# dcharatan/flowmap

Measured on NVIDIA B200. Metric: overfit iters/sec at 150x360x640 (149 frame pairs per iteration), higher is better.
Workload: dtype f32

## Files before the change

### flowmap_b200/csrc/fm_kernels.cu

```cuda
#include <cuda_runtime.h>
#include <stdio.h>
#include <string.h>
#include <stdlib.h>

#include "../../include/flowmap_b200.h"
#include "fm_host.h"
#include "fm_pixel.cuh"

namespace fm_host {
namespace {
thread_local char g_err[512] = "";
unsigned long long g_launches = 0;
}
int fail(const char* what, cudaError_t e) {
  snprintf(g_err, sizeof(g_err), "%s: %s", what, cudaGetErrorString(e));
  return 1;
}
int fail_msg(const char* what) {
  snprintf(g_err, sizeof(g_err), "%s", what);
  return 2;
}
void count_launch() { __atomic_add_fetch(&g_launches, 1, __ATOMIC_RELAXED); }
const char* last_error() { return g_err; }
unsigned long long launches() { return __atomic_load_n(&g_launches, __ATOMIC_RELAXED); }
// ... 1163 lines not shown
__device__ __forceinline__ Cam sm_cam(const float* rec) {
  Cam c;
  c.fx = rec1(rec, 15); c.fy = rec1(rec, 16); c.cx = rec1(rec, 17); c.cy = rec1(rec, 18);
  c.ifx = rec1(rec, 19); c.ify = rec1(rec, 20);
  return c;
}

template <int NT = kThreads>
__device__ __forceinline__ int block_compact(bool valid, int value, int* list, int* warp_base) {
  const int lane = threadIdx.x & 31, warp = threadIdx.x >> 5;
  const unsigned m = __ballot_sync(0xffffffffu, valid);
  if (lane == 0) warp_base[warp] = __popc(m);
  __syncthreads();
  int base = 0, total = 0;
#pragma unroll
  for (int w = 0; w < NT / 32; ++w) {
    const int c = warp_base[w];
    if (w < warp) base += c;
    total += c;
  }
  if (valid) list[base + __popc(m & ((1u << lane) - 1u))] = value;
  __syncthreads();
  return total;
}

struct TrackSlot { int slot; bool owner; };
template <int N, int OFF>
struct SlotWalk {
  __device__ __forceinline__ static void run(int lane, int& pos, bool& ok) {
    if (N == 1) {
      SlotWalk<1, OFF / 2>::run(lane, pos, ok);
      ok = ok && (lane & OFF) == 0;
    } else {
      constexpr int HALF = (N + 1) / 2;
      SlotWalk<HALF, OFF / 2>::run(lane, pos, ok);
      if (lane & OFF) pos += HALF;
      ok = ok && pos < N;
    }
  }
};
template <int N>
struct SlotWalk<N, 0> {
  __device__ __forceinline__ static void run(int, int& pos, bool& ok) { pos = 0; ok = true; }
};
template <int N>
__device__ __forceinline__ TrackSlot track_slot(int lane) {
  TrackSlot t;
  SlotWalk<N, 16>::run(lane, t.slot, t.owner);
  return t;
}
template <int N, int OFF>
__device__ __forceinline__ void halve_exchange(float* v, bool upper) {
  constexpr int HALF = (N + 1) / 2;
#pragma unroll
  for (int j = 0; j < HALF; ++j) {
    const float hi = (j + HALF < N) ? v[j + HALF] : 0.f;
    const float send = upper ? v[j] : hi;
    const float keep = upper ? hi : v[j];
    v[j] = keep + __shfl_xor_sync(0xffffffffu, send, OFF);
  }
}
template <int N, int OFF>
struct WarpSumN {
  __device__ __forceinline__ static void run(float* v, int lane) {
    if (N == 1) {
      v[0] += __shfl_xor_sync(0xffffffffu, v[0], OFF);
      WarpSumN<1, OFF / 2>::run(v, lane);
    } else {
      halve_exchange<N, OFF>(v, lane & OFF);
      WarpSumN<(N + 1) / 2, OFF / 2>::run(v, lane);
    }
  }
};
template <int N>
struct WarpSumN<N, 0> {
  __device__ __forceinline__ static void run(float*, int) {}
};
template <int N>
__device__ __forceinline__ float warp_sum_n(float* v, int lane) {
  WarpSumN<N, 16>::run(v, lane);
  return v[0];
}

constexpr int kTrackThreads = 128;
constexpr int kTrackPoints = 2 * kTrackThreads;

template <bool SHARED_K>
__global__ void __launch_bounds__(kTrackThreads, 5)
k_track_src(const float* __restrict__ depth, const float* __restrict__ k4, const float* __restrict__ ext,
            const int* __restrict__ seg, const float* __restrict__ txy,
            const unsigned char* __restrict__ tvis, int mapping, float delta, double* __restrict__ sums,
            unsigned char* __restrict__ flag, float* __restrict__ dq_out,
            double* __restrict__ trackacc, int H, int W, TrackShard sh) {
  extern __shared__ float sm[];
  constexpr int NW = kTrackThreads / 32;
  __shared__ double red[kTrackAcc * NW];
  const SegInfo si = load_seg(seg, blockIdx.z);
  const int row = blockIdx.y;
  if (row >= si.rows || !sh.owns(si.start_frame + row)) return;
  load_segment_frames(sm, ext, k4, si);
  float* s_tgt = sm + (size_t)gridDim.y * 2 * kTrackRec;
  __shared__ int s_list[kTrackPoints];
  __shared__ int s_wbase[NW];
  const GridDims grid = make_grid(H, W);
  const RobustCfg rc = make_robust(mapping, delta, H, W);
  const int frame = si.start_frame + row;
  const float* D = depth + (size_t)(frame - sh.depth_frame0) * H * W;
  const float* rsrec = sm + row * 2 * kTrackRec;
  float rs[12];
#pragma unroll
  for (int i = 0; i < 12; ++i) rs[i] = rec1(rsrec, i);
  const Cam ks = sm_cam(rsrec);
  const int lane = threadIdx.x & 31, warp = threadIdx.x >> 5;
  float acc[kTrackAcc], lc[2] = {0.f, 0.f};
#pragma unroll
  for (int i = 0; i < kTrackAcc; ++i) acc[i] = 0.f;
  int count = 0;
#pragma unroll
  for (int h = 0; h < 2; ++h) {
    const int p_own = blockIdx.x * kTrackPoints + h * kTrackThreads + (int)threadIdx.x;
    bool ok_own = false;
    if (p_own < si.n) {
      const size_t sidx = (size_t)si.sample_start + (size_t)row * si.n + p_own;
      const float2 sxy = __ldg(reinterpret_cast<const float2*>(txy) + sidx);
      ok_own = tvis[sidx] && in_unit_square(sxy.x, sxy.y);
      flag[sidx] = ok_own ? 1 : 0;
    }
    count += block_compact<kTrackThreads>(ok_own, p_own, s_list + count, s_wbase);
  }
  const int half = (count + 1) >> 1;
  const bool live_a = (int)threadIdx.x < half, live_b = (int)threadIdx.x + half < count;
  if (warp * 32 < half) {
    const int pa = live_a ? s_list[threadIdx.x] : 0, pb = live_b ? s_list[threadIdx.x + half] : 0;
    const size_t row0 = (size_t)si.sample_start + (size_t)row * si.n;
    float qa[3] = {0.f, 0.f, 0.f}, qb[3] = {0.f, 0.f, 0.f};
    F2 Xw[3] = {f2s(0.f), f2s(0.f), f2s(0.f)};
    auto lift = [&](int p, float* q, float* X) {
      const float2 sxy = __ldg(reinterpret_cast<const float2*>(txy) + row0 + p);
      const Taps t = bilinear_taps(sxy.x, sxy.y, grid);
      sample_surface(t, grid, ks, [D](int o) { return __ldg(D + o); }, q[0], q[1], q[2]);
#pragma unroll
      for (int i = 0; i < 3; ++i)
        X[i] = fm_fma(rs[i * 3 + 0], q[0], fm_fma(rs[i * 3 + 1], q[1], fm_fma(rs[i * 3 + 2], q[2], rs[9 + i])));
    };
    if (live_a) { float X[3]; lift(pa, qa, X); Xw[0].x = X[0]; Xw[1].x = X[1]; Xw[2].x = X[2]; }
    if (live_b) { float X[3]; lift(pb, qb, X); Xw[0].y = X[0]; Xw[1].y = X[1]; Xw[2].y = X[2]; }
    F2 G[3] = {f2s(0.f), f2s(0.f), f2s(0.f)}, lc2[2] = {f2s(0.f), f2s(0.f)};
    F2 kt[4] = {f2s(0.f), f2s(0.f), f2s(0.f), f2s(0.f)};
    constexpr int NRED = SHARED_K ? 6 : kTrackAcc;
    constexpr int SLOT0 = kTrackAcc - NRED;
    const TrackSlot slot = track_slot<NRED>(lane);
    float* tgt = s_tgt + (size_t)warp * si.rows * kTrackAcc;
    size_t ia = (size_t)si.sample_start + pa, ib = (size_t)si.sample_start + pb;
    unsigned char va_n = live_a ? tvis[ia] : 0, vb_n = live_b ? tvis[ib] : 0;
    float2 ga_n = live_a ? __ldg(reinterpret_cast<const float2*>(txy) + ia) : make_float2(0.f, 0.f);
    float2 gb_n = live_b ? __ldg(reinterpret_cast<const float2*>(txy) + ib) : make_float2(0.f, 0.f);
    for (int ft = 0; ft < si.rows; ++ft) {
      const unsigned char vis_a = va_n, vis_b = vb_n;
      const float2 ga = ga_n, gb = gb_n;
      if (ft + 1 < si.rows) {
        if (live_a) { ia += si.n; va_n = tvis[ia]; ga_n = __ldg(reinterpret_cast<const float2*>(txy) + ia); }
        if (live_b) { ib += si.n; vb_n = tvis[ib]; gb_n = __ldg(reinterpret_cast<const float2*>(txy) + ib); }
      }
      float c[NRED];
#pragma unroll
      for (int i = 0; i < NRED; ++i) c[i] = 0.f;
      bool ok = false;
      if (vis_a | vis_b) {
        const float* rec = sm + ft * 2 * kTrackRec;
        F2 R[9];
#pragma unroll
        for (int i = 0; i < 9; ++i) R[i] = rec2(rec, i);
        const F2 dir0 = f2_fma(R[0], Xw[0], f2_fma(R[3], Xw[1], f2_mul(R[6], Xw[2])));
        const F2 dir1 = f2_fma(R[1], Xw[0], f2_fma(R[4], Xw[1], f2_mul(R[7], Xw[2])));
        const F2 dir2 = f2_fma(R[2], Xw[0], f2_fma(R[5], Xw[1], f2_mul(R[8], Xw[2])));
        Cam2 kc;
        kc.fx = rec2(rec, 15); kc.fy = rec2(rec, 16); kc.cx = rec2(rec, 17); kc.cy = rec2(rec, 18);
        const LeanTerm2 lt = lean_term2(f2s(1.0f), dir0, dir1, dir2, rec2(rec, 12), rec2(rec, 13), rec2(rec, 14), kc,
                                        f2(ga.x, gb.x), f2(ga.y, gb.y), f2s(0.f), f2s(0.f), f2s(1.0f), rc);
        const bool oa = vis_a && in_unit_square(lt.uvx.x, lt.uvy.x);
        const bool ob = vis_b && in_unit_square(lt.uvx.y, lt.uvy.y);
        if (oa | ob) {
          ok = true;
          const F2 d0 = f2(oa ? lt.d0.x : 0.f, ob ? lt.d0.y : 0.f);
          const F2 d1 = f2(oa ? lt.d1.x : 0.f, ob ? lt.d1.y : 0.f);
          const F2 d2 = f2(oa ? lt.d2.x : 0.f, ob ? lt.d2.y : 0.f);
          lc2[0] = f2_add(lc2[0], f2(oa ? lt.loss.x : 0.f, ob ? lt.loss.y : 0.f));
          lc2[1] = f2_add(lc2[1], f2(oa ? 1.f : 0.f, ob ? 1.f : 0.f));
          const F2 g0 = f2_fma(R[0], d0, f2_fma(R[1], d1, f2_mul(R[2], d2)));
          const F2 g1 = f2_fma(R[3], d0, f2_fma(R[4], d1, f2_mul(R[5], d2)));
          const F2 g2 = f2_fma(R[6], d0, f2_fma(R[7], d1, f2_mul(R[8], d2)));
          G[0] = f2_add(G[0], g0); G[1] = f2_add(G[1], g1); G[2] = f2_add(G[2], g2);
          const F2 ex = f2_mul(d0, rec2(rec, 19)), ey = f2_mul(d1, rec2(rec, 20));
          if (SHARED_K) {
            kt[0] = f2_fma(ex, lt.P0, kt[0]); kt[1] = f2_fma(ey, lt.P1, kt[1]);
            kt[2] = f2_fma(ex, lt.P2, kt[2]); kt[3] = f2_fma(ey, lt.P2, kt[3]);
          } else {
            const F2 k0 = f2_mul(ex, lt.P0), k1 = f2_mul(ey, lt.P1), k2 = f2_mul(ex, lt.P2), k3 = f2_mul(ey, lt.P2);
            c[0] = k0.x + k0.y; c[1] = k1.x + k1.y; c[2] = k2.x + k2.y; c[3] = k3.x + k3.y;
          }
          const F2 e0 = f2_sub(Xw[0], rec2(rec, 9)), e1 = f2_sub(Xw[1], rec2(rec, 10)), e2 = f2_sub(Xw[2], rec2(rec, 11));
          const F2 t0 = f2_fma(e2, g1, f2_neg(f2_mul(e1, g2)));
          const F2 t1 = f2_fma(e0, g2, f2_neg(f2_mul(e2, g0)));
          const F2 t2 = f2_fma(e1, g0, f2_neg(f2_mul(e0, g1)));
          float* tw = c + (SHARED_K ? 0 : 4);
          tw[0] = t0.x + t0.y; tw[1] = t1.x + t1.y; tw[2] = t2.x + t2.y;
          tw[3] = -(g0.x + g0.y); tw[4] = -(g1.x + g1.y); tw[5] = -(g2.x + g2.y);
        }
      }
      float total = 0.f;
      if (__ballot_sync(0xffffffffu, ok)) total = warp_sum_n<NRED>(c, lane);
      if (slot.owner) tgt[ft * kTrackAcc + SLOT0 + slot.slot] = total;
    }
    lc[0] = lc2[0].x + lc2[0].y;
    lc[1] = lc2[1].x + lc2[1].y;
    auto finish = [&](int p, const float* q, float X0, float X1, float X2, float G0, float G1, float G2, float k0,
                      float k1, float k2, float k3) {
      const size_t sidx = row0 + p;
      const float dq0 = fm_fma(rs[0], G0, fm_fma(rs[3], G1, rs[6] * G2));
      const float dq1 = fm_fma(rs[1], G0, fm_fma(rs[4], G1, rs[7] * G2));
      const float dq2 = fm_fma(rs[2], G0, fm_fma(rs[5], G1, rs[8] * G2));
      dq_out[sidx * 3 + 0] = dq0; dq_out[sidx * 3 + 1] = dq1; dq_out[sidx * 3 + 2] = dq2;
      const float e0 = dq0 * ks.ifx, e1 = dq1 * ks.ify;
      acc[0] += k0 - e0 * q[0]; acc[1] += k1 - e1 * q[1]; acc[2] += k2 - e0 * q[2]; acc[3] += k3 - e1 * q[2];
      const float c0 = X0 - rs[9], c1 = X1 - rs[10], c2 = X2 - rs[11];
      acc[4] += c1 * G2 - c2 * G1;
      acc[5] += c2 * G0 - c0 * G2;
      acc[6] += c0 * G1 - c1 * G0;
      acc[7] += G0; acc[8] += G1; acc[9] += G2;
    };
    if (live_a) finish(pa, qa, Xw[0].x, Xw[1].x, Xw[2].x, G[0].x, G[1].x, G[2].x, kt[0].x, kt[1].x, kt[2].x, kt[3].x);
    if (live_b) finish(pb, qb, Xw[0].y, Xw[1].y, Xw[2].y, G[0].y, G[1].y, G[2].y, kt[0].y, kt[1].y, kt[2].y, kt[3].y);
  }
  block_accumulate<2, kTrackThreads>(lc, sums, red);
  block_accumulate<kTrackAcc, kTrackThreads>(acc, trackacc + (size_t)frame * kTrackAcc, red);
  const int live_warps = (half + 31) >> 5;
  for (int i = threadIdx.x; i < si.rows * kTrackAcc; i += kTrackThreads) {
    if (SHARED_K && i % kTrackAcc < 4) continue;
    double t = 0.0;
    for (int w = 0; w < live_warps; ++w) t += (double)s_tgt[(size_t)w * si.rows * kTrackAcc + i];
    if (t != 0.0) atomicAdd(trackacc + (size_t)si.start_frame * kTrackAcc + i, t);
  }
}

__device__ __forceinline__ double track_scale(const double* sums, float loss_weight, const float* go) {
  double cnt = sums[1];
  if (cnt == 0.0) cnt = 1.0;
  return (double)loss_weight * (go ? (double)*go : 1.0) / cnt;
}

__global__ void k_track_loss(const double* __restrict__ sums, float loss_weight, float* __restrict__ loss) {
  *loss = (float)(track_scale(sums, loss_weight, nullptr) * sums[0]);
}

__global__ void __launch_bounds__(kThreads)
k_track_apply(const float* __restrict__ k4, const int* __restrict__ seg, const float* __restrict__ txy,
              const unsigned char* __restrict__ flag, const float* __restrict__ dq,
              const double* __restrict__ sums, float loss_weight, const float* __restrict__ go,
              float* __restrict__ g_depth, int H, int W, TrackShard sh) {
  const SegInfo si = load_seg(seg, blockIdx.z);
  const int row = blockIdx.y;
  const int p = blockIdx.x * kThreads + threadIdx.x;
  if (row >= si.rows || p >= si.n || !sh.owns(si.start_frame + row)) return;
  const size_t sidx = (size_t)si.sample_start + (size_t)row * si.n + p;
  if (!flag[sidx]) return;
  const float scale = (float)track_scale(sums, loss_weight, go);
  const int frame = si.start_frame + row;
  const GridDims grid = make_grid(H, W);
  const Cam ks = make_cam(load_k4(k4, frame));
  const float2 sxy = __ldg(reinterpret_cast<const float2*>(txy) + sidx);
  const Taps t = bilinear_taps(sxy.x, sxy.y, grid);
  const float dq0 = scale * dq[sidx * 3 + 0], dq1 = scale * dq[sidx * 3 + 1], dq2 = scale * dq[sidx * 3 + 2];
  float rx0, ry0, rx1, ry1;
  tap_rays(t, grid, ks, rx0, ry0, rx1, ry1);
  float* gd = g_depth + (size_t)(frame - sh.depth_frame0) * H * W;
  red_add(gd + t.y0 * W + t.x0, t.w00 * (dq0 * rx0 + dq1 * ry0 + dq2));
  red_add(gd + t.y0 * W + t.x1, t.w01 * (dq0 * rx1 + dq1 * ry0 + dq2));
  red_add(gd + t.y1 * W + t.x0, t.w10 * (dq0 * rx0 + dq1 * ry1 + dq2));
  red_add(gd + t.y1 * W + t.x1, t.w11 * (dq0 * rx1 + dq1 * ry1 + dq2));
}

__global__ void k_track_finalize(const double* __restrict__ trackacc, const double* __restrict__ sums,
                                 float loss_weight, const float* __restrict__ go,
                                 const float* __restrict__ ext, float* __restrict__ g_ext,
                                 float* __restrict__ g_k4, int F) {
  const int f = blockIdx.x * blockDim.x + threadIdx.x;
  if (f >= F) return;
  const double sc = track_scale(sums, loss_weight, go);
  const double* a = trackacc + (size_t)f * kTrackAcc;
  for (int k = 0; k < 4; ++k) g_k4[(size_t)f * 4 + k] = (float)(sc * a[k]);
  const float* P = ext + (size_t)f * 16;
  const double w0 = 0.5 * sc * a[4], w1 = 0.5 * sc * a[5], w2 = 0.5 * sc * a[6];
  float* o = g_ext + (size_t)f * 16;
  for (int c = 0; c < 3; ++c) {
    const double r0 = P[0 * 4 + c], r1 = P[1 * 4 + c], r2 = P[2 * 4 + c];
    o[0 * 4 + c] = (float)(-w2 * r1 + w1 * r2);
    o[1 * 4 + c] = (float)(w2 * r0 - w0 * r2);
    o[2 * 4 + c] = (float)(-w1 * r0 + w0 * r1);
  }
  o[3] = (float)(sc * a[7]); o[7] = (float)(sc * a[8]); o[11] = (float)(sc * a[9]);
  o[12] = o[13] = o[14] = o[15] = 0.f;
}

constexpr int kSweepAcc = 80;

__global__ void k_sweep_base_k4(const float* __restrict__ cand_k4, float* __restrict__ base_k4, int B, int n) {
  const int t = blockIdx.x * blockDim.x + threadIdx.x;
  if (t >= B * 8) return;
  const int b = t >> 3, e = t & 7;
  base_k4[t] = cand_k4[(size_t)b * n * 8 + e];
}

__global__ void k_sweep_scale_solve(const double* __restrict__ base_moments, const float* __restrict__ depth,
                                    const float* __restrict__ cand_k4, float* __restrict__ rt,
                                    PairState* __restrict__ state, int B, int n, PairLayout lay, int H, int W) {
  const int item = blockIdx.x * blockDim.x + threadIdx.x;
  if (item >= B * n) return;
  const int b = item / n;
  const PairAddr pa = pair_addr(lay, item, H * W);
  const double z0 = (double)__ldg(depth + pa.depth_a + (size_t)H * W + (size_t)(H / 2) * W + W / 2);
  const double sx = (double)cand_k4[(size_t)b * n * 8 + 0] / (double)cand_k4[(size_t)item * 8 + 0];
  const double sy = (double)cand_k4[(size_t)b * n * 8 + 1] / (double)cand_k4[(size_t)item * 8 + 1];
  const double sc[3] = {sx, sy, 1.0};
  double m[kNumMoments];
  const double* bm = base_moments + (size_t)b * kNumMoments;
  m[0] = bm[0];
  for (int i = 0; i < 3; ++i) { m[1 + i] = bm[1 + i] * sc[i]; m[4 + i] = bm[4 + i] * sc[i]; }
  for (int a = 0; a < 3; ++a)
    for (int c = 0; c < 3; ++c) m[7 + a * 3 + c] = bm[7 + a * 3 + c] * sc[a] * sc[c];
  const double shift[3] = {0.0, 0.0, z0};
  PairState st;
  float out[12];
  procrustes_solve(m, shift, out, st);
  for (int k = 0; k < 12; ++k) rt[(size_t)item * 12 + k] = out[k];
  state[item] = st;
}

__global__ void k_sweep_aggregate(const PairAdjoint* __restrict__ adj, const float* __restrict__ cand_k4,
                                  PairAdjoint* __restrict__ out, int B, int n) {
  const int b = blockIdx.x, lane = threadIdx.x;
  double acc[16];
#pragma unroll
  for (int i = 0; i < 16; ++i) acc[i] = 0.0;
  for (int c = lane; c < n; c += 32) {
    const int item = b * n + c;
    const PairAdjoint a = adj[item];
    const double s[3] = {(double)cand_k4[(size_t)b * n * 8 + 0] / (double)cand_k4[(size_t)item * 8 + 0],
                         (double)cand_k4[(size_t)b * n * 8 + 1] / (double)cand_k4[(size_t)item * 8 + 1], 1.0};
// ... 770 lines not shown
  cudaStream_t s = (cudaStream_t)stream;
  Workspace w = carve(ws, B, F);
  const int BP = B * (F - 1), BF = B * F;
  cudaError_t e = cudaMemsetAsync(w.flowacc, 0, (size_t)BF * kFlowAcc * sizeof(double), s);
  if (e != cudaSuccess) return fail("fm_flow_loss_fwd_bwd: memset", e);
  int rc = launch_flow(depth, k4, rt, forward_flow, backward_flow, forward_mask, backward_mask, mask_sum,
                       mapping, delta, loss_weight, intrinsics_mode, g_depth, w.flowacc, B, F, H, W, s);
  if (rc) return rc;
  const int n = BF > BP ? BF : BP;
  k_flow_finalize<<<(n + 127) / 128, 128, 0, s>>>(w.flowacc, rt, loss, g_rt, g_k4, B, F);
  FM_CHECK_LAUNCH("fm_flow_loss_fwd_bwd: k_flow_finalize");
  return 0;
}

int fm_pose_chain(const float* rt, float* extrinsics, int B, int F, void* stream) {
  if (!rt || !extrinsics || B < 1 || F < 2) return fail_msg("fm_pose_chain: bad arguments");
  k_pose_chain<<<B, kChainThreads, 0, (cudaStream_t)stream>>>(rt, extrinsics, B, F);
  FM_CHECK_LAUNCH("fm_pose_chain");
  return 0;
}

int fm_pose_chain_bwd(const float* rt, const float* extrinsics, const float* g_extrinsics, float* g_rt,
                      int B, int F, void* stream) {
  if (!rt || !extrinsics || !g_extrinsics || !g_rt || B < 1 || F < 2) return fail_msg("fm_pose_chain_bwd: bad arguments");
  k_pose_chain_bwd<<<B, kChainThreads, 0, (cudaStream_t)stream>>>(rt, extrinsics, g_extrinsics, g_rt, B, F);
  FM_CHECK_LAUNCH("fm_pose_chain_bwd");
  return 0;
}

int fm_step_clock_tick(void* clock, double lr, double beta1, double beta2, unsigned long long base_seed,
                       int tick_focal, void* stream) {
  if (!clock) return fail_msg("fm_step_clock_tick: bad arguments");
  k_clock_tick<<<1, 1, 0, (cudaStream_t)stream>>>((StepClock*)clock, lr, beta1, beta2, base_seed, tick_focal);
  FM_CHECK_LAUNCH("fm_step_clock_tick");
  return 0;
}

int fm_adam_step_clock(float* param, const float* grad, float* exp_avg, float* exp_avg_sq, size_t count,
                       const void* clock, int focal_clock, double beta1_d, double beta2_d, double eps_d,
                       void* stream) {
  if (!param || !grad || !exp_avg || !exp_avg_sq || !clock) return fail_msg("fm_adam_step_clock: bad arguments");
  if (count == 0) return 0;
  size_t nb = (count / 4 + kThreads * 2 - 1) / (kThreads * 2);
  if (nb < 1) nb = 1;
  if (nb > 148 * 16) nb = 148 * 16;
  const StepClock* c = (const StepClock*)clock;
  k_adam<<<(unsigned)nb, kThreads, 0, (cudaStream_t)stream>>>(
      param, grad, exp_avg, exp_avg_sq, count, (float)beta1_d, (float)beta2_d, (float)(1.0 - beta1_d),
      (float)(1.0 - beta2_d), (float)eps_d, 0.f, 1.f, focal_clock ? &c->focal_step_size : &c->step_size);
  FM_CHECK_LAUNCH("fm_adam_step_clock");
  return 0;
}

int fm_random_subset_clock(const void* clock, long long N, int n, int64_t* out, void* stream) {
  if (!clock || N < 1 || n < 1 || n > N || !out) return fail_msg("fm_random_subset_clock: bad arguments");
  k_random_subset<<<(n + 127) / 128, 128, 0, (cudaStream_t)stream>>>(0ull, N, n, out, &((const StepClock*)clock)->seed);
  FM_CHECK_LAUNCH("fm_random_subset_clock");
  return 0;
}

int fm_adam_step(float* param, const float* grad, float* exp_avg, float* exp_avg_sq, size_t count,
                 double lr, double beta1_d, double beta2_d, double eps_d, int step, void* stream) {
  if (!param || !grad || !exp_avg || !exp_avg_sq || step < 1) return fail_msg("fm_adam_step: bad arguments");
  if (count == 0) return 0;
  const float beta1 = (float)beta1_d, beta2 = (float)beta2_d, eps = (float)eps_d;
  const double bc1 = 1.0 - pow(beta1_d, (double)step);
  const double bc2 = 1.0 - pow(beta2_d, (double)step);
  const float step_size = (float)(lr / bc1);
  const float bc2_sqrt = (float)sqrt(bc2);
  size_t nb = (count / 4 + kThreads * 2 - 1) / (kThreads * 2);
  if (nb < 1) nb = 1;
  if (nb > 148 * 16) nb = 148 * 16;
  k_adam<<<(unsigned)nb, kThreads, 0, (cudaStream_t)stream>>>(param, grad, exp_avg, exp_avg_sq, count, beta1, beta2, (float)(1.0 - (double)beta1_d), (float)(1.0 - (double)beta2_d), eps, step_size, bc2_sqrt);
  FM_CHECK_LAUNCH("fm_adam_step");
  return 0;
}

size_t fm_track_workspace_bytes(int F, long long total_samples) {
  if (F < 1 || total_samples < 0) return 0;
  size_t off = 0;
  off = align_up(off + 4 * sizeof(double), 256);
  off = align_up(off + (size_t)F * kTrackAcc * sizeof(double), 256);
  off = align_up(off + (size_t)total_samples * 3 * sizeof(float), 256);
  off = align_up(off + (size_t)total_samples, 256);
  return off;
}

namespace {
struct TrackWs { double* sums; double* acc; float* dq; unsigned char* flag; };
TrackWs carve_track(void* base, int F, long long total) {
  char* p = (char*)base; size_t off = 0; TrackWs w;
  w.sums = (double*)(p + off); off = align_up(off + 4 * sizeof(double), 256);
  w.acc = (double*)(p + off); off = align_up(off + (size_t)F * kTrackAcc * sizeof(double), 256);
  w.dq = (float*)(p + off); off = align_up(off + (size_t)total * 3 * sizeof(float), 256);
  w.flag = (unsigned char*)(p + off);
  return w;
}
}

size_t fm_track_reduce_bytes(int F) {
  if (F < 1) return 0;
  return align_up(4 * sizeof(double), 256) + align_up((size_t)F * kTrackAcc * sizeof(double), 256);
}

int fm_track_loss_fwd_sharded(const float* depth, const float* k4, const float* extrinsics, const int* segments,
                              int num_segments, int max_rows, int max_points, const float* track_xy,
                              const unsigned char* track_vis, long long total_samples, int mapping, float delta,
                              float loss_weight, float* loss, void* ws, int F, int H, int W, int depth_frame0,
                              int src_frame_lo, int src_frame_hi, int shared_intrinsics, void* stream) {
  if (!depth || !k4 || !extrinsics || !segments || !track_xy || !track_vis || !ws ||
      num_segments < 1 || max_rows < 1 || max_points < 1 || F < 1)
    return fail_msg("fm_track_loss_fwd: bad arguments");
  if (mapping < 0 || mapping > 2) return fail_msg("fm_track_loss_fwd: unknown mapping");
  if (depth_frame0 < 0 || src_frame_lo < depth_frame0 || src_frame_hi > F || src_frame_lo > src_frame_hi)
    return fail_msg("fm_track_loss_fwd: bad source-frame range");
  cudaStream_t s = (cudaStream_t)stream;
  TrackWs w = carve_track(ws, F, total_samples);
  cudaError_t e = cudaMemsetAsync(w.sums, 0, (char*)w.dq - (char*)w.sums, s);
  if (e != cudaSuccess) return fail("fm_track_loss_fwd: memset", e);
  dim3 grid((max_points + kTrackPoints - 1) / kTrackPoints, max_rows, num_segments);
  const size_t smem = (size_t)max_rows * (2 * kTrackRec + (kTrackThreads / 32) * kTrackAcc) * sizeof(float);
  if (smem > 200 * 1024) return fail_msg("fm_track_loss_fwd: segment too long for shared memory");
  if (smem > 48 * 1024) {
    cudaError_t ea = shared_intrinsics
        ? cudaFuncSetAttribute(k_track_src<true>, cudaFuncAttributeMaxDynamicSharedMemorySize, (int)smem)
        : cudaFuncSetAttribute(k_track_src<false>, cudaFuncAttributeMaxDynamicSharedMemorySize, (int)smem);
    if (ea != cudaSuccess) return fail("fm_track_loss_fwd: shared memory", ea);
  }
  const TrackShard sh = {depth_frame0, src_frame_lo, src_frame_hi};
  if (shared_intrinsics)
    k_track_src<true><<<grid, kTrackThreads, smem, s>>>(depth, k4, extrinsics, segments, track_xy, track_vis, mapping,
                                                  delta, w.sums, w.flag, w.dq, w.acc, H, W, sh);
  else
    k_track_src<false><<<grid, kTrackThreads, smem, s>>>(depth, k4, extrinsics, segments, track_xy, track_vis, mapping,
                                                   delta, w.sums, w.flag, w.dq, w.acc, H, W, sh);
  FM_CHECK_LAUNCH("fm_track_loss_fwd: k_track_src");
  if (loss) {
    k_track_loss<<<1, 1, 0, s>>>(w.sums, loss_weight, loss);
    FM_CHECK_LAUNCH("fm_track_loss_fwd: k_track_loss");
  }
  return 0;
}

int fm_track_loss_fwd(const float* depth, const float* k4, const float* extrinsics, const int* segments,
                      int num_segments, int max_rows, int max_points, const float* track_xy,
                      const unsigned char* track_vis, long long total_samples, int mapping, float delta,
                      float loss_weight, float* loss, void* ws, int F, int H, int W, void* stream) {
  if (!loss) return fail_msg("fm_track_loss_fwd: bad arguments");
  return fm_track_loss_fwd_sharded(depth, k4, extrinsics, segments, num_segments, max_rows, max_points, track_xy,
                                   track_vis, total_samples, mapping, delta, loss_weight, loss, ws, F, H, W, 0,
                                   0, F, 0, stream);
}

int fm_track_loss_value(const void* ws, float loss_weight, float* loss, void* stream) {
  if (!ws || !loss) return fail_msg("fm_track_loss_value: bad arguments");
  k_track_loss<<<1, 1, 0, (cudaStream_t)stream>>>((const double*)ws, loss_weight, loss);
  FM_CHECK_LAUNCH("fm_track_loss_value");
  return 0;
}

static int track_bwd_impl(const float* k4, const float* extrinsics, const int* segments, int num_segments,
                          int max_rows, int max_points, const float* track_xy, long long total_samples,
                          float loss_weight, const float* grad_out, float* g_depth, float* g_extrinsics,
                          float* g_k4, void* ws, int F, int H, int W, int depth_frame0, int src_frame_lo,
                          int src_frame_hi, cudaStream_t s, cudaStream_t apply_stream) {
  if (!k4 || !extrinsics || !segments || !track_xy || !g_depth || !g_extrinsics || !g_k4 || !ws ||
      num_segments < 1 || max_rows < 1 || max_points < 1 || F < 1)
    return fail_msg("fm_track_loss_bwd: bad arguments");
  if (depth_frame0 < 0 || src_frame_lo < depth_frame0 || src_frame_hi > F || src_frame_lo > src_frame_hi)
    return fail_msg("fm_track_loss_bwd: bad source-frame range");
  TrackWs w = carve_track(ws, F, total_samples);
  dim3 grid((max_points + kThreads - 1) / kThreads, max_rows, num_segments);
  const TrackShard sh = {depth_frame0, src_frame_lo, src_frame_hi};
  k_track_apply<<<grid, kThreads, 0, apply_stream>>>(k4, segments, track_xy, w.flag, w.dq, w.sums, loss_weight,
                                                    grad_out, g_depth, H, W, sh);
  FM_CHECK_LAUNCH("fm_track_loss_bwd: k_track_apply");
  k_track_finalize<<<(F + 63) / 64, 64, 0, s>>>(w.acc, w.sums, loss_weight, grad_out, extrinsics, g_extrinsics,
                                               g_k4, F);
  FM_CHECK_LAUNCH("fm_track_loss_bwd: k_track_finalize");
  return 0;
}

int fm_track_loss_bwd_sharded(const float* depth, const float* k4, const float* extrinsics, const int* segments,
                              int num_segments, int max_rows, int max_points, const float* track_xy,
                              const unsigned char* track_vis, long long total_samples, int mapping, float delta,
                              float loss_weight, const float* grad_out, float* g_depth, float* g_extrinsics,
                              float* g_k4, void* ws, int F, int H, int W, int depth_frame0, int src_frame_lo,
                              int src_frame_hi, void* stream) {
  (void)depth; (void)track_vis; (void)mapping; (void)delta;
  return track_bwd_impl(k4, extrinsics, segments, num_segments, max_rows, max_points, track_xy, total_samples,
                        loss_weight, grad_out, g_depth, g_extrinsics, g_k4, ws, F, H, W, depth_frame0,
                        src_frame_lo, src_frame_hi, (cudaStream_t)stream, (cudaStream_t)stream);
}

int fm_track_loss_bwd(const float* depth, const float* k4, const float* extrinsics, const int* segments,
                      int num_segments, int max_rows, int max_points, const float* track_xy,
                      const unsigned char* track_vis, long long total_samples, int mapping, float delta,
                      float loss_weight, const float* grad_out, float* g_depth, float* g_extrinsics,
                      float* g_k4, void* ws, int F, int H, int W, void* stream) {
  return fm_track_loss_bwd_sharded(depth, k4, extrinsics, segments, num_segments, max_rows, max_points, track_xy,
                                   track_vis, total_samples, mapping, delta, loss_weight, grad_out, g_depth,
                                   g_extrinsics, g_k4, ws, F, H, W, 0, 0, F, stream);
}

size_t fm_points_workspace_bytes(int items) {
  if (items < 1) return 0;
  return carve(nullptr, items, 2).bytes;
}

int fm_align_rigid_fwd(const float* p, const float* q, const float* weights, float* rt, void* ws, int items,
                       int n, void* stream) {
  if (!p || !q || !weights || !rt || !ws || items < 1 || n < 1) return fail_msg("fm_align_rigid_fwd: bad arguments");
  cudaStream_t s = (cudaStream_t)stream;
  Workspace w = carve(ws, items, 2);
  cudaError_t e = cudaMemsetAsync(w.moments, 0, (size_t)items * kNumMoments * sizeof(double), s);
  if (e != cudaSuccess) return fail("fm_align_rigid_fwd: memset", e);
  dim3 grid(blocks_for(n, 1), items);
  k_points_moments<<<grid, kThreads, 0, s>>>(p, q, weights, w.moments, n);
  FM_CHECK_LAUNCH("fm_align_rigid_fwd: k_points_moments");
  k_points_solve<<<(items + 63) / 64, 64, 0, s>>>(w.moments, rt, w.state, items);
  FM_CHECK_LAUNCH("fm_align_rigid_fwd: k_points_solve");
  return 0;
}

int fm_align_rigid_bwd(const float* p, const float* q, const float* weights, const float* g_rt, float* g_p,
                       float* g_q, float* g_w, void* ws, int items, int n, void* stream) {
  if (!p || !q || !weights || !g_rt || !g_p || !g_q || !g_w || !ws || items < 1 || n < 1)
    return fail_msg("fm_align_rigid_bwd: bad arguments");
  cudaStream_t s = (cudaStream_t)stream;
  Workspace w = carve(ws, items, 2);
  k_adjoint<<<(items + 63) / 64, 64, 0, s>>>(w.flowacc, w.state, g_rt, 0, nullptr, w.adj, items, 2);
  FM_CHECK_LAUNCH("fm_align_rigid_bwd: k_adjoint");
  dim3 grid(blocks_for(n, 1), items);
  k_points_distribute<<<grid, kThreads, 0, s>>>(p, q, weights, w.adj, g_p, g_q, g_w, n);
  FM_CHECK_LAUNCH("fm_align_rigid_bwd: k_points_distribute");
  return 0;
}

int fm_unproject_points(const float* xy, const float* z, const float* k4, float* out, int items, int n,
                        int xy_shared, void* stream) {
  if (!xy || !z || !k4 || !out || items < 1 || n < 1) return fail_msg("fm_unproject_points: bad arguments");
  dim3 grid(blocks_for(n, 1), items);
  k_unproject_points<<<grid, kThreads, 0, (cudaStream_t)stream>>>(xy, z, k4, out, n, xy_shared);
  FM_CHECK_LAUNCH("fm_unproject_points");
  return 0;
}

int fm_unproject_points_bwd(const float* xy, const float* z, const float* k4, const float* g_out, float* g_z,
                            float* g_k4, void* ws, int items, int n, int xy_shared, void* stream) {
  if (!xy || !z || !k4 || !g_out || !g_z || !g_k4 || !ws || items < 1 || n < 1)
    return fail_msg("fm_unproject_points_bwd: bad arguments");
  cudaStream_t s = (cudaStream_t)stream;
  Workspace w = carve(ws, items, 2);
  cudaError_t e = cudaMemsetAsync(w.k4acc, 0, (size_t)items * 4 * sizeof(double), s);
  if (e != cudaSuccess) return fail("fm_unproject_points_bwd: memset", e);
  dim3 grid(blocks_for(n, 1), items);
  k_unproject_points_bwd<<<grid, kThreads, 0, s>>>(xy, z, k4, g_out, g_z, w.k4acc, n, xy_shared);
  FM_CHECK_LAUNCH("fm_unproject_points_bwd: k_unproject_points_bwd");
// ... 92 lines not shown
  FM_CHECK_LAUNCH("fm_softmin_sweep_bwd: k_sweep");
  k_sweep_out<<<(items * 12 + 127) / 128, 128, 0, s>>>(w.flowacc, g_rt, items, 1, 12);
  FM_CHECK_LAUNCH("fm_softmin_sweep_bwd: k_sweep_out");
  k_adjoint<<<(items + 63) / 64, 64, 0, s>>>(w.flowacc, w.state, g_rt, 0, nullptr, w.adj, items, 2);
  FM_CHECK_LAUNCH("fm_softmin_sweep_bwd: k_adjoint");
  k_sweep_aggregate<<<B, 32, 0, s>>>(w.adj, cand_k4, w.adj + items, B, num_candidates);
  FM_CHECK_LAUNCH("fm_softmin_sweep_bwd: k_sweep_aggregate");
  AdamFuse af;
  memset(&af, 0, sizeof(af));
  dim3 grid1(blocks_for_points(num_indices), B);
  k_distribute<1><<<grid1, kThreads, 0, s>>>(depth, base_k4, backward_flow, const_cast<float*>(weights), indices,
                                            num_indices, w.adj + items, g_depth, g_weights, w.k4acc,
                                            weight_sensitivity, lay1, af, H, W);
  FM_CHECK_LAUNCH("fm_softmin_sweep_bwd: k_distribute");
  return 0;
}

int fm_softmin_focal(const float* err, const float* cand_focal, int num_candidates, int B, float* softmin,
                     float* focal, void* stream) {
  if (!err || !cand_focal || !softmin || !focal || B < 1 || num_candidates < 1)
    return fail_msg("fm_softmin_focal: bad arguments");
  k_softmin_focal<<<B, 32, 0, (cudaStream_t)stream>>>(err, cand_focal, num_candidates, softmin, focal);
  FM_CHECK_LAUNCH("fm_softmin_focal");
  return 0;
}

int fm_softmin_focal_bwd(const float* softmin, const float* cand_focal, const float* focal,
                         const float* g_focal, int num_candidates, int B, float* g_err, void* stream) {
  if (!softmin || !cand_focal || !focal || !g_focal || !g_err || B < 1 || num_candidates < 1)
    return fail_msg("fm_softmin_focal_bwd: bad arguments");
  const int n = B * num_candidates;
  k_softmin_focal_bwd<<<(n + 127) / 128, 128, 0, (cudaStream_t)stream>>>(softmin, cand_focal, focal, g_focal,
                                                                        num_candidates, B, g_err);
  FM_CHECK_LAUNCH("fm_softmin_focal_bwd");
  return 0;
}

struct SideLane { cudaStream_t stream; cudaEvent_t fork, join; int state; };
static SideLane* side_lane() {
  static thread_local SideLane lanes[64];
  int dev = -1;
  if (cudaGetDevice(&dev) != cudaSuccess || dev < 0 || dev >= 64) return nullptr;
  SideLane& l = lanes[dev];
  if (l.state == 0) {
    const bool ok = cudaStreamCreateWithFlags(&l.stream, cudaStreamNonBlocking) == cudaSuccess &&
                    cudaEventCreateWithFlags(&l.fork, cudaEventDisableTiming) == cudaSuccess &&
                    cudaEventCreateWithFlags(&l.join, cudaEventDisableTiming) == cudaSuccess;
    l.state = ok ? 1 : -1;
    if (!ok) (void)cudaGetLastError();
  }
  return l.state == 1 ? &l : nullptr;
}

int fm_overfit_step(const fm_overfit_step_args* a, void* stream) {
  if (!a || !a->depth || !a->fflow || !a->bflow || !a->fmask || !a->bmask || !a->mask_sum ||
      !a->g_depth || !a->rt || !a->loss || !a->ws || !a->k4 || bad_dims(1, a->F, a->H, a->W))
    return fail_msg("fm_overfit_step: bad arguments");
  if (a->weight_logits && !a->g_weights) return fail_msg("fm_overfit_step: g_weights missing");
  if (a->tracks && (!a->extrinsics || !a->g_extrinsics || !a->track_ws || !a->track_loss))
    return fail_msg("fm_overfit_step: tracking needs extrinsics / g_extrinsics / track_ws / track_loss");
  cudaStream_t s = (cudaStream_t)stream;
  const int F = a->F, H = a->H, W = a->W, BP = F - 1;
  const size_t N = (size_t)H * W;
  Workspace w = carve(a->ws, 1, F);
  int rc;
  cudaError_t e;
  if (a->phase < FM_STEP_ALL || a->phase > FM_STEP_BACKWARD) return fail_msg("fm_overfit_step: unknown phase");
  void* plan = (a->splat_plan && !a->indices && tiled_shape_ok(F, H, W)) ? a->splat_plan : nullptr;
  float* k4 = a->k4;
  if (a->phase != FM_STEP_BACKWARD) {
    if (a->focal) {
      k_k4_from_focal<<<(F + 63) / 64, 64, 0, s>>>(a->focal, k4, F, H, W);
      FM_CHECK_LAUNCH("fm_overfit_step: k_k4_from_focal");
    }
    if ((rc = procrustes_fwd_impl(a->depth, k4, a->bflow, a->weight_logits, a->weight_sensitivity,
                                  a->indices, a->num_indices, a->rt, a->ws, 1, F, H, W, stream, nullptr, plan,
                                  (a->indices || plan) ? nullptr : a->moments_k4)))
      return rc;
    SideLane* fwd_lane = a->tracks ? side_lane() : nullptr;
    if (fwd_lane) {
      if ((e = cudaEventRecord(fwd_lane->fork, s)) != cudaSuccess) return fail("fm_overfit_step: fork", e);
      if ((e = cudaStreamWaitEvent(fwd_lane->stream, fwd_lane->fork, 0)) != cudaSuccess) return fail("fm_overfit_step: fork", e);
    }
    e = cudaMemsetAsync(w.flowacc, 0, (size_t)F * kFlowAcc * sizeof(double), s);
    if (e != cudaSuccess) return fail("fm_overfit_step: memset", e);
    if ((rc = launch_flow(a->depth, k4, a->rt, a->fflow, a->bflow, a->fmask, a->bmask, a->mask_sum,
                          a->mapping, a->delta, a->flow_weight, a->focal ? 1 : 2, a->g_depth, w.flowacc, 1, F,
                          H, W, s)))
      return rc;
    k_flow_finalize<<<(F + 127) / 128, 128, 0, s>>>(w.flowacc, a->rt, a->loss, nullptr, nullptr, 1, F);
    FM_CHECK_LAUNCH("fm_overfit_step: k_flow_finalize");
    if (a->tracks) {
      const fm_packed_tracks* t = a->tracks;
      void* ts = fwd_lane ? (void*)fwd_lane->stream : stream;
      if ((rc = fm_pose_chain(a->rt, a->extrinsics, 1, F, ts))) return rc;
      if ((rc = fm_track_loss_fwd_sharded(a->depth, k4, a->extrinsics, t->segments, t->num_segments, t->max_rows,
                                          t->max_points, t->xy, t->vis, t->total_samples, a->mapping, a->delta,
                                          a->track_weight, a->track_loss, a->track_ws, F, H, W, 0, 0, F, 1, ts)))
        return rc;
      if (fwd_lane) {
        if ((e = cudaEventRecord(fwd_lane->join, fwd_lane->stream)) != cudaSuccess) return fail("fm_overfit_step: join", e);
        if ((e = cudaStreamWaitEvent(s, fwd_lane->join, 0)) != cudaSuccess) return fail("fm_overfit_step: join", e);
      }
    }
  }
  if (a->phase == FM_STEP_FORWARD) return 0;
  const float* fscale = a->phase == FM_STEP_BACKWARD ? a->flow_grad_scale : nullptr;
  const float* tscale = a->phase == FM_STEP_BACKWARD ? a->track_grad_scale : nullptr;
  if (fscale) {
    k_scale_inplace<<<148 * 4, kThreads, 0, s>>>(a->g_depth, fscale, (size_t)F * N);
    FM_CHECK_LAUNCH("fm_overfit_step: k_scale_inplace");
  }
  const float* g_rt = a->phase == FM_STEP_BACKWARD ? a->g_rt : nullptr;
  const float* track_g_k4 = a->phase == FM_STEP_BACKWARD ? a->track_g_k4 : nullptr;
  SideLane* lane = nullptr;
  if (a->tracks) {
    const fm_packed_tracks* t = a->tracks;
    if (!plan) lane = side_lane();
    cudaStream_t apply_stream = s;
    if (lane) {
      if ((e = cudaEventRecord(lane->fork, s)) != cudaSuccess) return fail("fm_overfit_step: fork", e);
      if ((e = cudaStreamWaitEvent(lane->stream, lane->fork, 0)) != cudaSuccess) return fail("fm_overfit_step: fork", e);
      apply_stream = lane->stream;
    }
    if ((rc = track_bwd_impl(k4, a->extrinsics, t->segments, t->num_segments, t->max_rows, t->max_points, t->xy,
                             t->total_samples, a->track_weight, tscale, a->g_depth, a->g_extrinsics, a->track_g_k4,
                             a->track_ws, F, H, W, 0, 0, F, s, apply_stream)))
      return rc;
    if (lane && (e = cudaEventRecord(lane->join, lane->stream)) != cudaSuccess) return fail("fm_overfit_step: join", e);
    if ((rc = fm_pose_chain_bwd(a->rt, a->extrinsics, a->g_extrinsics, a->g_rt, 1, F, stream))) return rc;
    g_rt = a->g_rt;
    track_g_k4 = a->track_g_k4;
  }
  if (a->indices && a->g_weights) {
    e = cudaMemsetAsync(a->g_weights, 0, (size_t)BP * N * sizeof(float), s);
    if (e != cudaSuccess) return fail("fm_overfit_step: memset g_weights", e);
  }
  AdamFuse af;
  memset(&af, 0, sizeof(af));
  const bool defer = a->defer_adam != 0;
  const bool fuse_w = a->step > 0 && a->weight_logits && !a->indices && W % 4 == 0;
  const StepClock* clock = (const StepClock*)a->clock;
  if (fuse_w) {
    af.consts = clock ? &clock->step_size : nullptr;
    af.on = 1; af.m = a->m_weights; af.v = a->v_weights;
    af.first_pair = a->defer_adam == 1 ? 1 : 0;
    af.beta1 = (float)a->beta1; af.beta2 = (float)a->beta2;
    af.omb1 = (float)(1.0 - a->beta1); af.omb2 = (float)(1.0 - a->beta2); af.eps = (float)a->eps;
    af.step_size = (float)(a->lr / (1.0 - pow(a->beta1, (double)a->step)));
    af.bc2_sqrt = (float)sqrt(1.0 - pow(a->beta2, (double)a->step));
  }
  if ((rc = procrustes_bwd_impl(a->depth, k4, a->bflow, a->weight_logits, a->weight_sensitivity,
                                a->indices, a->num_indices, g_rt, 1, fscale, a->g_depth, a->g_weights,
                                a->g_k4, a->ws, 1, F, H, W, stream, nullptr, fuse_w ? &af : nullptr, plan,
                                a->splat_overflow_max, fscale != nullptr)))
    return rc;
  if (lane && (e = cudaStreamWaitEvent(s, lane->join, 0)) != cudaSuccess) return fail("fm_overfit_step: join", e);
  if (a->step > 0 && !defer) {
    auto adam = [&](float* p, const float* g, float* m, float* v, size_t n, int step, int focal_clock) -> int {
      return clock ? fm_adam_step_clock(p, g, m, v, n, clock, focal_clock, a->beta1, a->beta2, a->eps, stream)
                   : fm_adam_step(p, g, m, v, n, a->lr, a->beta1, a->beta2, a->eps, step, stream);
    };
    if ((rc = adam(a->depth, a->g_depth, a->m_depth, a->v_depth, (size_t)F * N, a->step, 0))) return rc;
    if (a->weight_logits && !fuse_w &&
        (rc = adam(a->weight_logits, a->g_weights, a->m_weights, a->v_weights, (size_t)BP * N, a->step, 0)))
      return rc;
    if (a->focal) {
      k_focal_grad<<<1, 256, 0, s>>>(w.k4acc, w.flowacc, track_g_k4, a->g_focal, 1, F, H, W, fscale);
      FM_CHECK_LAUNCH("fm_overfit_step: k_focal_grad");
      if ((rc = adam(a->focal, a->g_focal, a->m_focal, a->v_focal, 1, a->focal_step > 0 ? a->focal_step : a->step, 1)))
        return rc;
    }
  } else if (a->focal) {
    k_focal_grad<<<1, 256, 0, s>>>(w.k4acc, w.flowacc, track_g_k4, a->g_focal, 1, F, H, W, fscale);
    FM_CHECK_LAUNCH("fm_overfit_step: k_focal_grad");
  }
  if (defer && a->step > 0 && a->weight_logits && !fuse_w) return fail_msg("fm_overfit_step: defer_adam needs the fused weight update");
  return 0;
}

}
// ... 1 lines not shown
```

Before: 592.8.

## Compact visible track points in a plan kernel and assign fixed-size warp units

Adds a separate planning kernel that compacts visible, in-bounds track samples per row into an index list with per-row counts, replacing the per-block flag compaction. The source kernel then maps each warp to a 64-point unit found by a prefix scan over row counts, so blocks carry only live work instead of padded rows. Warp results are reduced in shared memory and flushed with atomics per frame. The apply kernel iterates the compacted list rather than testing flags. In the overfit step the plan is launched early on the side stream so it can overlap the flow loss. This adds an extra launch, atomics and a per-warp row search, and the intermediate rs/ks reload suggests register pressure.

```diff
diff --git a/flowmap_b200/csrc/fm_kernels.cu b/flowmap_b200/csrc/fm_kernels.cu
--- a/flowmap_b200/csrc/fm_kernels.cu
+++ b/flowmap_b200/csrc/fm_kernels.cu
@@ -1269,57 +1269,99 @@
   return v[0];
 }
 
+constexpr int kPlanThreads = 256;
+__global__ void __launch_bounds__(kPlanThreads)
+k_track_plan(const int* __restrict__ seg, const float* __restrict__ txy, const unsigned char* __restrict__ tvis,
+             int* __restrict__ list, int* __restrict__ rowcnt, TrackShard sh) {
+  __shared__ int s_wbase[kPlanThreads / 32];
+  const SegInfo si = load_seg(seg, blockIdx.y);
+  const int row = blockIdx.x;
+  if (row >= si.rows || si.n < 1) return;
+  const size_t row0 = (size_t)si.sample_start + (size_t)row * si.n;
+  int count = 0;
+  if (sh.owns(si.start_frame + row)) {
+    for (int base = 0; base < si.n; base += kPlanThreads) {
+      const int p = base + (int)threadIdx.x;
+      bool ok = false;
+      if (p < si.n) {
+        const float2 sxy = __ldg(reinterpret_cast<const float2*>(txy) + row0 + p);
+        ok = tvis[row0 + p] && in_unit_square(sxy.x, sxy.y);
+      }
+      count += block_compact<kPlanThreads>(ok, p, list + row0 + count, s_wbase);
+    }
+  }
+  if (threadIdx.x == 0) rowcnt[si.sample_start + row] = count;
+}
+
 constexpr int kTrackThreads = 128;
-constexpr int kTrackPoints = 2 * kTrackThreads;
+constexpr int kTrackUnit = 64;
+
+struct TrackUnit { int row, off, cnt, total; };
+__device__ __forceinline__ TrackUnit find_unit(const int* rowcnt, const SegInfo& si, int k, int lane) {
+  TrackUnit u = {-1, 0, 0, 0};
+  for (int r0 = 0; r0 < si.rows; r0 += 32) {
+    const int r = r0 + lane;
+    const int c = r < si.rows ? __ldg(rowcnt + si.sample_start + r) : 0;
+    const int nu = (c + kTrackUnit - 1) / kTrackUnit;
+    int incl = nu;
+#pragma unroll
+    for (int o = 1; o < 32; o <<= 1) {
+      const int t = __shfl_up_sync(0xffffffffu, incl, o);
+      if (lane >= o) incl += t;
+    }
+    const int first = u.total + incl - nu;
+    if (k >= first && k < first + nu) { u.row = r; u.off = (k - first) * kTrackUnit; u.cnt = min(kTrackUnit, c - u.off); }
+    u.total += __shfl_sync(0xffffffffu, incl, 31);
+  }
+  const unsigned m = __ballot_sync(0xffffffffu, u.row >= 0);
+  if (m) {
+    const int src = __ffs(m) - 1;
+    u.row = __shfl_sync(0xffffffffu, u.row, src);
+    u.off = __shfl_sync(0xffffffffu, u.off, src);
+    u.cnt = __shfl_sync(0xffffffffu, u.cnt, src);
+  }
+  return u;
+}
 
 template <bool SHARED_K>
 __global__ void __launch_bounds__(kTrackThreads, 5)
 k_track_src(const float* __restrict__ depth, const float* __restrict__ k4, const float* __restrict__ ext,
             const int* __restrict__ seg, const float* __restrict__ txy,
             const unsigned char* __restrict__ tvis, int mapping, float delta, double* __restrict__ sums,
-            unsigned char* __restrict__ flag, float* __restrict__ dq_out,
+            const int* __restrict__ list, const int* __restrict__ rowcnt, float* __restrict__ dq_out,
             double* __restrict__ trackacc, int H, int W, TrackShard sh) {
   extern __shared__ float sm[];
   constexpr int NW = kTrackThreads / 32;
-  __shared__ double red[kTrackAcc * NW];
-  const SegInfo si = load_seg(seg, blockIdx.z);
-  const int row = blockIdx.y;
-  if (row >= si.rows || !sh.owns(si.start_frame + row)) return;
+  constexpr int NSRC = 2 + kTrackAcc;
+  __shared__ float s_src[NW][NSRC];
+  __shared__ int s_frame[NW];
+  const SegInfo si = load_seg(seg, blockIdx.y);
+  if (si.n < 1) return;
+  const int lane = threadIdx.x & 31, warp = threadIdx.x >> 5;
+  const TrackUnit u = find_unit(rowcnt, si, (int)blockIdx.x * NW + warp, lane);
+  if ((int)blockIdx.x * NW >= u.total) return;
+  if (lane == 0) s_frame[warp] = u.row >= 0 ? si.start_frame + u.row : -1;
   load_segment_frames(sm, ext, k4, si);
-  float* s_tgt = sm + (size_t)gridDim.y * 2 * kTrackRec;
-  __shared__ int s_list[kTrackPoints];
-  __shared__ int s_wbase[NW];
-  const GridDims grid = make_grid(H, W);
-  const RobustCfg rc = make_robust(mapping, delta, H, W);
-  const int frame = si.start_frame + row;
-  const float* D = depth + (size_t)(frame - sh.depth_frame0) * H * W;
-  const float* rsrec = sm + row * 2 * kTrackRec;
-  float rs[12];
-#pragma unroll
-  for (int i = 0; i < 12; ++i) rs[i] = rec1(rsrec, i);
-  const Cam ks = sm_cam(rsrec);
-  const int lane = threadIdx.x & 31, warp = threadIdx.x >> 5;
+  float* s_tgt = sm + (size_t)si.rows * 2 * kTrackRec;
   float acc[kTrackAcc], lc[2] = {0.f, 0.f};
 #pragma unroll
   for (int i = 0; i < kTrackAcc; ++i) acc[i] = 0.f;
-  int count = 0;
-#pragma unroll
-  for (int h = 0; h < 2; ++h) {
-    const int p_own = blockIdx.x * kTrackPoints + h * kTrackThreads + (int)threadIdx.x;
-    bool ok_own = false;
-    if (p_own < si.n) {
-      const size_t sidx = (size_t)si.sample_start + (size_t)row * si.n + p_own;
-      const float2 sxy = __ldg(reinterpret_cast<const float2*>(txy) + sidx);
-      ok_own = tvis[sidx] && in_unit_square(sxy.x, sxy.y);
-      flag[sidx] = ok_own ? 1 : 0;
-    }
-    count += block_compact<kTrackThreads>(ok_own, p_own, s_list + count, s_wbase);
-  }
-  const int half = (count + 1) >> 1;
-  const bool live_a = (int)threadIdx.x < half, live_b = (int)threadIdx.x + half < count;
-  if (warp * 32 < half) {
-    const int pa = live_a ? s_list[threadIdx.x] : 0, pb = live_b ? s_list[threadIdx.x + half] : 0;
+  if (u.row >= 0) {
+    const int row = u.row, count = u.cnt;
+    const GridDims grid = make_grid(H, W);
+    const RobustCfg rc = make_robust(mapping, delta, H, W);
+    const int frame = si.start_frame + row;
+    const float* D = depth + (size_t)(frame - sh.depth_frame0) * H * W;
+    const float* rsrec = sm + row * 2 * kTrackRec;
+    float rs[12];
+#pragma unroll
+    for (int i = 0; i < 12; ++i) rs[i] = rec1(rsrec, i);
+    Cam ks = sm_cam(rsrec);
     const size_t row0 = (size_t)si.sample_start + (size_t)row * si.n;
+    const int half = (count + 1) >> 1;
+    const bool live_a = lane < half, live_b = lane + half < count;
+    const int* ul = list + row0 + u.off;
+    const int pa = live_a ? __ldg(ul + lane) : 0, pb = live_b ? __ldg(ul + lane + half) : 0;
     float qa[3] = {0.f, 0.f, 0.f}, qb[3] = {0.f, 0.f, 0.f};
     F2 Xw[3] = {f2s(0.f), f2s(0.f), f2s(0.f)};
     auto lift = [&](int p, float* q, float* X) {
@@ -1401,6 +1443,9 @@
     }
     lc[0] = lc2[0].x + lc2[0].y;
     lc[1] = lc2[1].x + lc2[1].y;
+#pragma unroll
+    for (int i = 0; i < 12; ++i) rs[i] = rec1(rsrec, i);
+    ks = sm_cam(rsrec);
     auto finish = [&](int p, const float* q, float X0, float X1, float X2, float G0, float G1, float G2, float k0,
                       float k1, float k2, float k3) {
       const size_t sidx = row0 + p;
@@ -1419,9 +1464,31 @@
     if (live_a) finish(pa, qa, Xw[0].x, Xw[1].x, Xw[2].x, G[0].x, G[1].x, G[2].x, kt[0].x, kt[1].x, kt[2].x, kt[3].x);
     if (live_b) finish(pb, qb, Xw[0].y, Xw[1].y, Xw[2].y, G[0].y, G[1].y, G[2].y, kt[0].y, kt[1].y, kt[2].y, kt[3].y);
   }
-  block_accumulate<2, kTrackThreads>(lc, sums, red);
-  block_accumulate<kTrackAcc, kTrackThreads>(acc, trackacc + (size_t)frame * kTrackAcc, red);
-  const int live_warps = (half + 31) >> 5;
+  {
+    float v[NSRC];
+    v[0] = lc[0]; v[1] = lc[1];
+#pragma unroll
+    for (int i = 0; i < kTrackAcc; ++i) v[2 + i] = acc[i];
+    const TrackSlot slot = track_slot<NSRC>(lane);
+    const float t = warp_sum_n<NSRC>(v, lane);
+    if (slot.owner) s_src[warp][slot.slot] = t;
+  }
+  __syncthreads();
+  if (threadIdx.x < NSRC) {
+    const int i = threadIdx.x;
+    double t = 0.0;
+    for (int w = 0; w < NW && s_frame[w] >= 0; ++w) {
+      t += (double)s_src[w][i];
+      if (i < 2) continue;
+      if (w + 1 == NW || s_frame[w + 1] != s_frame[w]) {
+        atomicAdd(trackacc + (size_t)s_frame[w] * kTrackAcc + (i - 2), t);
+        t = 0.0;
+      }
+    }
+    if (i < 2) atomicAdd(sums + i, t);
+  }
+  int live_warps = 0;
+  while (live_warps < NW && s_frame[live_warps] >= 0) ++live_warps;
   for (int i = threadIdx.x; i < si.rows * kTrackAcc; i += kTrackThreads) {
     if (SHARED_K && i % kTrackAcc < 4) continue;
     double t = 0.0;
@@ -1442,15 +1509,15 @@
 
 __global__ void __launch_bounds__(kThreads)
 k_track_apply(const float* __restrict__ k4, const int* __restrict__ seg, const float* __restrict__ txy,
-              const unsigned char* __restrict__ flag, const float* __restrict__ dq,
+              const int* __restrict__ list, const int* __restrict__ rowcnt, const float* __restrict__ dq,
               const double* __restrict__ sums, float loss_weight, const float* __restrict__ go,
               float* __restrict__ g_depth, int H, int W, TrackShard sh) {
   const SegInfo si = load_seg(seg, blockIdx.z);
   const int row = blockIdx.y;
-  const int p = blockIdx.x * kThreads + threadIdx.x;
-  if (row >= si.rows || p >= si.n || !sh.owns(si.start_frame + row)) return;
-  const size_t sidx = (size_t)si.sample_start + (size_t)row * si.n + p;
-  if (!flag[sidx]) return;
+  const int i = blockIdx.x * kThreads + threadIdx.x;
+  if (row >= si.rows || si.n < 1 || i >= __ldg(rowcnt + si.sample_start + row)) return;
+  const size_t row0 = (size_t)si.sample_start + (size_t)row * si.n;
+  const size_t sidx = row0 + __ldg(list + row0 + i);
   const float scale = (float)track_scale(sums, loss_weight, go);
   const int frame = si.start_frame + row;
   const GridDims grid = make_grid(H, W);
@@ -2387,18 +2454,20 @@
   off = align_up(off + 4 * sizeof(double), 256);
   off = align_up(off + (size_t)F * kTrackAcc * sizeof(double), 256);
   off = align_up(off + (size_t)total_samples * 3 * sizeof(float), 256);
-  off = align_up(off + (size_t)total_samples, 256);
+  off = align_up(off + (size_t)total_samples * sizeof(int), 256);
+  off = align_up(off + (size_t)total_samples * sizeof(int), 256);
   return off;
 }
 
 namespace {
-struct TrackWs { double* sums; double* acc; float* dq; unsigned char* flag; };
+struct TrackWs { double* sums; double* acc; float* dq; int* list; int* rowcnt; };
 TrackWs carve_track(void* base, int F, long long total) {
   char* p = (char*)base; size_t off = 0; TrackWs w;
   w.sums = (double*)(p + off); off = align_up(off + 4 * sizeof(double), 256);
   w.acc = (double*)(p + off); off = align_up(off + (size_t)F * kTrackAcc * sizeof(double), 256);
   w.dq = (float*)(p + off); off = align_up(off + (size_t)total * 3 * sizeof(float), 256);
-  w.flag = (unsigned char*)(p + off);
+  w.list = (int*)(p + off); off = align_up(off + (size_t)total * sizeof(int), 256);
+  w.rowcnt = (int*)(p + off);
   return w;
 }
 }
@@ -2408,11 +2477,21 @@
   return align_up(4 * sizeof(double), 256) + align_up((size_t)F * kTrackAcc * sizeof(double), 256);
 }
 
-int fm_track_loss_fwd_sharded(const float* depth, const float* k4, const float* extrinsics, const int* segments,
-                              int num_segments, int max_rows, int max_points, const float* track_xy,
-                              const unsigned char* track_vis, long long total_samples, int mapping, float delta,
-                              float loss_weight, float* loss, void* ws, int F, int H, int W, int depth_frame0,
-                              int src_frame_lo, int src_frame_hi, int shared_intrinsics, void* stream) {
+static int track_plan(const int* segments, int num_segments, int max_rows, const float* track_xy,
+                      const unsigned char* track_vis, long long total_samples, void* ws, int F, TrackShard sh,
+                      cudaStream_t s) {
+  TrackWs w = carve_track(ws, F, total_samples);
+  k_track_plan<<<dim3(max_rows, num_segments), kPlanThreads, 0, s>>>(segments, track_xy, track_vis, w.list, w.rowcnt,
+                                                                    sh);
+  FM_CHECK_LAUNCH("fm_track_loss_fwd: k_track_plan");
+  return 0;
+}
+
+static int track_fwd_impl(const float* depth, const float* k4, const float* extrinsics, const int* segments,
+                          int num_segments, int max_rows, int max_points, const float* track_xy,
+                          const unsigned char* track_vis, long long total_samples, int mapping, float delta,
+                          float loss_weight, float* loss, void* ws, int F, int H, int W, int depth_frame0,
+                          int src_frame_lo, int src_frame_hi, int shared_intrinsics, bool run_plan, void* stream) {
   if (!depth || !k4 || !extrinsics || !segments || !track_xy || !track_vis || !ws ||
       num_segments < 1 || max_rows < 1 || max_points < 1 || F < 1)
     return fail_msg("fm_track_loss_fwd: bad arguments");
@@ -2423,7 +2502,13 @@
   TrackWs w = carve_track(ws, F, total_samples);
   cudaError_t e = cudaMemsetAsync(w.sums, 0, (char*)w.dq - (char*)w.sums, s);
   if (e != cudaSuccess) return fail("fm_track_loss_fwd: memset", e);
-  dim3 grid((max_points + kTrackPoints - 1) / kTrackPoints, max_rows, num_segments);
+  const TrackShard sh = {depth_frame0, src_frame_lo, src_frame_hi};
+  int rc;
+  if (run_plan &&
+      (rc = track_plan(segments, num_segments, max_rows, track_xy, track_vis, total_samples, ws, F, sh, s)))
+    return rc;
+  const long long units = (long long)max_rows * ((max_points + kTrackUnit - 1) / kTrackUnit);
+  dim3 grid((unsigned)((units + kTrackThreads / 32 - 1) / (kTrackThreads / 32)), num_segments);
   const size_t smem = (size_t)max_rows * (2 * kTrackRec + (kTrackThreads / 32) * kTrackAcc) * sizeof(float);
   if (smem > 200 * 1024) return fail_msg("fm_track_loss_fwd: segment too long for shared memory");
   if (smem > 48 * 1024) {
@@ -2432,19 +2517,28 @@
         : cudaFuncSetAttribute(k_track_src<false>, cudaFuncAttributeMaxDynamicSharedMemorySize, (int)smem);
     if (ea != cudaSuccess) return fail("fm_track_loss_fwd: shared memory", ea);
   }
-  const TrackShard sh = {depth_frame0, src_frame_lo, src_frame_hi};
   if (shared_intrinsics)
     k_track_src<true><<<grid, kTrackThreads, smem, s>>>(depth, k4, extrinsics, segments, track_xy, track_vis, mapping,
-                                                  delta, w.sums, w.flag, w.dq, w.acc, H, W, sh);
+                                                  delta, w.sums, w.list, w.rowcnt, w.dq, w.acc, H, W, sh);
   else
     k_track_src<false><<<grid, kTrackThreads, smem, s>>>(depth, k4, extrinsics, segments, track_xy, track_vis, mapping,
-                                                   delta, w.sums, w.flag, w.dq, w.acc, H, W, sh);
+                                                   delta, w.sums, w.list, w.rowcnt, w.dq, w.acc, H, W, sh);
   FM_CHECK_LAUNCH("fm_track_loss_fwd: k_track_src");
   if (loss) {
     k_track_loss<<<1, 1, 0, s>>>(w.sums, loss_weight, loss);
     FM_CHECK_LAUNCH("fm_track_loss_fwd: k_track_loss");
   }
   return 0;
+}
+
+int fm_track_loss_fwd_sharded(const float* depth, const float* k4, const float* extrinsics, const int* segments,
+                              int num_segments, int max_rows, int max_points, const float* track_xy,
+                              const unsigned char* track_vis, long long total_samples, int mapping, float delta,
+                              float loss_weight, float* loss, void* ws, int F, int H, int W, int depth_frame0,
+                              int src_frame_lo, int src_frame_hi, int shared_intrinsics, void* stream) {
+  return track_fwd_impl(depth, k4, extrinsics, segments, num_segments, max_rows, max_points, track_xy, track_vis,
+                        total_samples, mapping, delta, loss_weight, loss, ws, F, H, W, depth_frame0, src_frame_lo,
+                        src_frame_hi, shared_intrinsics, true, stream);
 }
 
 int fm_track_loss_fwd(const float* depth, const float* k4, const float* extrinsics, const int* segments,
@@ -2477,8 +2571,8 @@
   TrackWs w = carve_track(ws, F, total_samples);
   dim3 grid((max_points + kThreads - 1) / kThreads, max_rows, num_segments);
   const TrackShard sh = {depth_frame0, src_frame_lo, src_frame_hi};
-  k_track_apply<<<grid, kThreads, 0, apply_stream>>>(k4, segments, track_xy, w.flag, w.dq, w.sums, loss_weight,
-                                                    grad_out, g_depth, H, W, sh);
+  k_track_apply<<<grid, kThreads, 0, apply_stream>>>(k4, segments, track_xy, w.list, w.rowcnt, w.dq, w.sums,
+                                                    loss_weight, grad_out, g_depth, H, W, sh);
   FM_CHECK_LAUNCH("fm_track_loss_bwd: k_track_apply");
   k_track_finalize<<<(F + 63) / 64, 64, 0, s>>>(w.acc, w.sums, loss_weight, grad_out, extrinsics, g_extrinsics,
                                                g_k4, F);
@@ -2737,6 +2831,15 @@
       if ((e = cudaEventRecord(fwd_lane->fork, s)) != cudaSuccess) return fail("fm_overfit_step: fork", e);
       if ((e = cudaStreamWaitEvent(fwd_lane->stream, fwd_lane->fork, 0)) != cudaSuccess) return fail("fm_overfit_step: fork", e);
     }
+    if (a->tracks) {
+      const fm_packed_tracks* t = a->tracks;
+      if (!t->segments || !t->xy || !t->vis || t->num_segments < 1 || t->max_rows < 1)
+        return fail_msg("fm_overfit_step: bad tracks");
+      const TrackShard all = {0, 0, F};
+      if ((rc = track_plan(t->segments, t->num_segments, t->max_rows, t->xy, t->vis, t->total_samples, a->track_ws, F,
+                           all, fwd_lane ? fwd_lane->stream : s)))
+        return rc;
+    }
     e = cudaMemsetAsync(w.flowacc, 0, (size_t)F * kFlowAcc * sizeof(double), s);
     if (e != cudaSuccess) return fail("fm_overfit_step: memset", e);
     if ((rc = launch_flow(a->depth, k4, a->rt, a->fflow, a->bflow, a->fmask, a->bmask, a->mask_sum,
@@ -2749,9 +2852,9 @@
       const fm_packed_tracks* t = a->tracks;
       void* ts = fwd_lane ? (void*)fwd_lane->stream : stream;
       if ((rc = fm_pose_chain(a->rt, a->extrinsics, 1, F, ts))) return rc;
-      if ((rc = fm_track_loss_fwd_sharded(a->depth, k4, a->extrinsics, t->segments, t->num_segments, t->max_rows,
-                                          t->max_points, t->xy, t->vis, t->total_samples, a->mapping, a->delta,
-                                          a->track_weight, a->track_loss, a->track_ws, F, H, W, 0, 0, F, 1, ts)))
+      if ((rc = track_fwd_impl(a->depth, k4, a->extrinsics, t->segments, t->num_segments, t->max_rows,
+                               t->max_points, t->xy, t->vis, t->total_samples, a->mapping, a->delta,
+                               a->track_weight, a->track_loss, a->track_ws, F, H, W, 0, 0, F, 1, false, ts)))
         return rc;
       if (fwd_lane) {
         if ((e = cudaEventRecord(fwd_lane->join, fwd_lane->stream)) != cudaSuccess) return fail("fm_overfit_step: join", e);
```

New measurement: 599.2, median of 6. +1.1%, better.
